# fgnt/pb_bss

Measured on NVIDIA H100. Metric: EM iterations/s, cACGMM F=513 T=500 D=8 K=3 (100-iteration fit), higher is better.
Workload: dtype f64

## Files before the change

### pb_bss_b200/csrc/em_persistent.cuh

```cuda
#pragma once
#include "common.cuh"
#include "em_kernels.cuh"
#include "heig.cuh"

namespace pbb {

#ifdef PBB_PHASE_TIMING
#define PBB_PH(i) do { if (tid == 0) { long long _t = clock64(); atomicAdd(&a.phase[i], (unsigned long long)(_t - _tp)); _tp = _t; } } while (0)
#else
#define PBB_PH(i) do { } while (0)
#endif

struct PersistArgs {
  const void* z;
  int zs;
  int F, T;
  int iterations;
  int first_is_m;
  int user_model;
  int softmax_fast;
  const double* aff_in;
  const double* saliency;
  const uint8_t* activity;
  double aff_eps;
  double eigenvalue_floor;
  int covariance_norm;
  int weight_mode;
  double* coef;
  double* ld;
  double* w;
  double* ew;
  double* part;
  int* flags;
  int* ticket;
  const int* dead;
  int* status;
  CwSpline spline;
  int wave_c;
  int wait_load;
  const int* order;
  unsigned long long* phase;
  int tsplit;
  double* tpart;
  int* tcount;
};

__device__ __forceinline__ uint32_t smem_u32(const void* p) {
  return static_cast<uint32_t>(__cvta_generic_to_shared(p));
}
__device__ __forceinline__ void mbar_init(uint64_t* bar, int count) {
  asm volatile("mbarrier.init.shared::cta.b64 [%0], %1;" ::"r"(smem_u32(bar)), "r"(count) : "memory");
}
__device__ __forceinline__ void mbar_expect_tx(uint64_t* bar, uint32_t bytes) {
  asm volatile("mbarrier.arrive.expect_tx.shared::cta.b64 _, [%0], %1;" ::"r"(smem_u32(bar)), "r"(bytes)
               : "memory");
}
__device__ __forceinline__ void mbar_wait(uint64_t* bar, uint32_t parity) {
  asm volatile(
      "{\n"
      ".reg .pred p;\n"
      "WAIT_%=:\n"
      "mbarrier.try_wait.parity.shared::cta.b64 p, [%0], %1;\n"
      "@p bra DONE_%=;\n"
      "bra WAIT_%=;\n"
      "DONE_%=:\n"
      "}\n" ::"r"(smem_u32(bar)),
      "r"(parity)
      : "memory");
}
__device__ __forceinline__ void bulk_g2s(void* dst, const void* src, uint32_t bytes, uint64_t* bar) {
  asm volatile("cp.async.bulk.shared::cluster.global.mbarrier::complete_tx::bytes [%0], [%1], %2, [%3];" ::"r"(
                   smem_u32(dst)),
               "l"(src), "r"(bytes), "r"(smem_u32(bar))
               : "memory");
}

constexpr int kStageFrames = 128;

template <int D, typename CT>
__device__ __forceinline__ void stage_g2s(CT (*dst)[kStageFrames], const CT* z, int bin, int nchunks, int chunk,
                                          uint64_t* bar) {
  constexpr int ROWS = stage_rows(D);
  constexpr uint32_t kRowBytes = kStageFrames * sizeof(CT);
  const CT* src = z + ((size_t)bin * nchunks + chunk) * (D * kStageFrames);
  mbar_expect_tx(bar, ROWS * kRowBytes);
  bulk_g2s(dst[0], src, D * kRowBytes, bar);
#pragma unroll
  for (int r = D; r < ROWS; ++r) bulk_g2s(dst[r], src + row_channel(D, r) * kStageFrames, kRowBytes, bar);
}

__device__ __forceinline__ int ld_acquire_gpu(const int* p) {
  int v;
  asm volatile("ld.acquire.gpu.global.s32 %0, [%1];" : "=r"(v) : "l"(p) : "memory");
  return v;
}
__device__ __forceinline__ void st_release_gpu(int* p, int v) {
  asm volatile("st.release.gpu.global.s32 [%0], %1;" ::"l"(p), "r"(v) : "memory");
}
__device__ __forceinline__ double fast_rcp(double x) {
  double r;
  asm("rcp.approx.ftz.f64 %0, %1;" : "=d"(r) : "d"(x));
  double e = fma(-x, r, 1.0);
  r = fma(r, e, r);
  e = fma(-x, r, 1.0);
  r = fma(r, e, r);
  return r;
}

__device__ __forceinline__ long long wave_h(long long r, int F, int c) {
  const long long m = F / c;
  const long long n = r < m ? r : m;
  return (long long)c * n * (n + 1) / 2 + (r - n) * (long long)F;
}
__device__ __forceinline__ long long wave_prefix(int r, int F, int I, int c) {
  return wave_h(r, F, c) - wave_h(r > I ? r - I : 0, F, c);
}
__device__ __forceinline__ void decode_ticket(int t, int F, int I, int c, int& bin, int& it) {
  if (c == 0) {
    it = t / F;
    bin = t - it * F;
    return;
  }
  int lo = 0, hi = I + (F + c - 1) / c - 1;
  while (hi - lo > 1) {
    const int mid = (lo + hi) >> 1;
    if (wave_prefix(mid, F, I, c) <= (long long)t) lo = mid; else hi = mid;
  }
  const long long first = (long long)c * (lo - I + 1 > 0 ? lo - I + 1 : 0);
  bin = (int)(first < F ? first : F) + (int)(t - wave_prefix(lo, F, I, c));
  it = lo - bin / c;
}
__device__ __forceinline__ int order_entry(const PersistArgs& a, int t, int S) {
  return a.order != nullptr ? __ldcg(a.order + t / S) : 0;
}
__device__ __forceinline__ void decode_task(const PersistArgs& a, int t, int S, int ord, int& bin, int& it, int& part) {
  const int tt = t / S;
  part = t - tt * S;
  if (a.order != nullptr) {
    bin = ord & 0xffff;
    it = ord >> 16;
  } else {
    decode_ticket(tt, a.F, a.iterations, a.wave_c, bin, it);
  }
}

__device__ __forceinline__ double2 lds_cplx(const double2* p) { return *p; }
__device__ __forceinline__ double2 lds_cplx(const float2* p) {
  const float2 v = *p;
  return make_double2((double)v.x, (double)v.y);
}

constexpr int kStages = 2;

template <int D, int K, typename CT>
struct PersistSmem {
  static constexpr int NS = D * D;
  static constexpr int M = D / 2;
  static constexpr int ROWS = stage_rows(D);
  CT zbuf[kStages][ROWS][kStageFrames];
  double2 A[K][NS];
  double2 V[K][NS];
  double2 W[K][NS];
  double coef[2][K][NS];
  double xq[2][M][2 * K][32];
  double S[K][NS + 1];
  alignas(16) double rot[K][((D + 1) / 2) * 6];
  double lam[K][D];
  double ld[K], w[K];
  alignas(16) double ew[2][4];
  alignas(16) double raw[2][8];
  uint64_t full[kStages];
  int tab[NS];
  int tick[8];
  int ready;
};

template <int D>
struct GroupDims {
  static constexpr int NSG = group_shape(D).nsg, NLOC = group_shape(D).nloc, NS = D * D;
  static constexpr int NFULL = group_shape(D).nfull, HALF = group_shape(D).half, M = D / 2;
};

template <int D>
__device__ __forceinline__ void group_psi(const double2 (&x)[GroupDims<D>::NLOC], double (&psi)[GroupDims<D>::NSG]) {
  using G = GroupDims<D>;
  psi[0] = x[0].x * x[0].x + x[0].y * x[0].y;
  psi[1] = x[1].x * x[1].x + x[1].y * x[1].y;
  psi[2] = x[0].x * x[1].x + x[0].y * x[1].y;
  psi[3] = x[0].x * x[1].y - x[0].y * x[1].x;
#pragma unroll
  for (int j = 0; j < G::NFULL; ++j) {
#pragma unroll
    for (int q = 0; q < 4; ++q) {
      const double2 u = x[q / 2], v = x[2 + 2 * j + (q % 2)];
      psi[4 + 8 * j + 2 * q] = u.x * v.x + u.y * v.y;
      psi[4 + 8 * j + 2 * q + 1] = u.x * v.y - u.y * v.x;
    }
  }
  if (G::HALF) {
#pragma unroll
    for (int h = 0; h < 2; ++h) {
      const double2 u = x[h], v = x[2 + 2 * G::NFULL + h];
      psi[4 + 8 * G::NFULL + 2 * h] = u.x * v.x + u.y * v.y;
      psi[4 + 8 * G::NFULL + 2 * h + 1] = u.x * v.y - u.y * v.x;
    }
  }
}

template <int D, int K>
__device__ __forceinline__ void softmax_product(double (&q)[K], const double* __restrict__ ew, double eps,
                                                double (&gam)[K], double (&cw)[K]) {
  const bool dead = q[0] < 1e-200;
#pragma unroll
  for (int k = 0; k < K; ++k) q[k] = dead ? 1.0 : q[k];
  double P[K];
  if constexpr (K == 2) {
    P[0] = q[1]; P[1] = q[0];
  } else if constexpr (K == 3) {
    P[0] = q[1] * q[2]; P[1] = q[0] * q[2]; P[2] = q[0] * q[1];
  } else {
    const double q01 = q[0] * q[1], q23 = q[2] * q[3];
    P[0] = q[1] * q23; P[1] = q[0] * q23; P[2] = q01 * q[3]; P[3] = q01 * q[2];
  }
  double b[K];
  double S = 1e-300;
#pragma unroll
  for (int k = 0; k < K; ++k) {
    b[k] = ew[k] * ipow<D>(P[k]);
    S += b[k];
  }
  const double rS = fast_rcp(S);
  const double rQ = fast_rcp(q[0] * P[0]);
  const double hi = 1.0 - eps;
#pragma unroll
  for (int k = 0; k < K; ++k) {
    double g = b[k] * rS;
    if (eps != 0.0) {
      g = g < eps ? eps : g;
      g = g > hi ? hi : g;
    }
    gam[k] = g;
    cw[k] = g * (P[k] * rQ);
  }
}

template <int K>
__device__ __forceinline__ void softmax_watson(const double (&q)[K], const double* __restrict__ kappa,
                                               const double* __restrict__ lognorm, const double* __restrict__ w,
                                               double (&gam)[K], double (&cw)[K]) {
  double lp[K];
  double m = -INFINITY;
#pragma unroll
  for (int k = 0; k < K; ++k) {
    lp[k] = fma(kappa[k], q[k], -lognorm[k]);
    m = lp[k] > m ? lp[k] : m;
  }
  double den = 0.0;
#pragma unroll
  for (int k = 0; k < K; ++k) {
    gam[k] = exp(lp[k] - m) * w[k];
    den += gam[k];
  }
  const double inv = 1.0 / fmax(den, kTiny);
#pragma unroll
  for (int k = 0; k < K; ++k) {
    gam[k] *= inv;
    cw[k] = gam[k];
  }
}

template <int D, bool NAMED>
__device__ __forceinline__ void em_exchange_barrier() {
  if constexpr (NAMED) asm volatile("bar.sync 1, %0;" ::"n"(32 * (D / 2)) : "memory");
  else __syncthreads();
}

template <int D, int K, int FR, typename CT>
__device__ __forceinline__ void lean_partial_forms(const CT* __restrict__ zrow, const double* __restrict__ cg,
                                                   double* __restrict__ xw, double (&psi)[FR][GroupDims<D>::NSG]) {
  using G = GroupDims<D>;
  constexpr int NSG = G::NSG, NLOC = G::NLOC, NS = G::NS;
  {
    double2 x[NLOC];
#pragma unroll
    for (int f = 0; f < FR; ++f) {
#pragma unroll
      for (int l = 0; l < NLOC; ++l) x[l] = lds_cplx(zrow + l * kStageFrames + 32 * f);
      group_psi<D>(x, psi[f]);
    }
  }
  double p0[FR][K], p1[FR][K];
#pragma unroll
  for (int k = 0; k < K; ++k)
#pragma unroll
    for (int f = 0; f < FR; ++f) { p0[f][k] = 0.0; p1[f][k] = 0.0; }
#pragma unroll
  for (int i = 0; i < NSG; i += 2) {
#pragma unroll
    for (int k = 0; k < K; ++k) {
      const double2 cc = *reinterpret_cast<const double2*>(cg + k * NS + i);
#pragma unroll
      for (int f = 0; f < FR; ++f) p0[f][k] = fma(cc.x, psi[f][i], p0[f][k]);
#pragma unroll
      for (int f = 0; f < FR; ++f) p1[f][k] = fma(cc.y, psi[f][i + 1], p1[f][k]);
    }
  }
#pragma unroll
  for (int k = 0; k < K; ++k)
#pragma unroll
    for (int f = 0; f < FR; ++f) xw[(f * K + k) * 32] = p0[f][k] + p1[f][k];
}

template <int D, int K, typename CT, int MODEL, bool NAMED = false, typename SMT>
__device__ __forceinline__ void lean_step(SMT& sm, int cb, int g, int st, int j, int lane, int& buf, double eps,
                                          double (&acc)[K * GroupDims<D>::NSG], double (&sg)[K]) {
  using G = GroupDims<D>;
  constexpr int NSG = G::NSG, M = G::M;
  double psi[1][NSG];
  lean_partial_forms<D, K, 1, CT>(&sm.zbuf[st][2 * g][0] + lane + 32 * j, &sm.coef[cb][0][g * NSG],
                                  &sm.xq[buf][g][0][lane], psi);
  em_exchange_barrier<D, NAMED>();
  const double* __restrict__ xr = &sm.xq[buf][0][0][lane];
  double q[K];
#pragma unroll
  for (int k = 0; k < K; ++k) {
    double v = xr[k * 32];
#pragma unroll
    for (int gg = 1; gg < M; ++gg) v += xr[(gg * 2 * K + k) * 32];
    q[k] = fabs(v);
  }
  buf ^= 1;
  double gam[K], cw[K];
  if constexpr (MODEL == 1) softmax_watson<K>(q, sm.ew[cb], sm.ld, sm.w, gam, cw);
  else softmax_product<D, K>(q, sm.ew[cb], eps, gam, cw);
#pragma unroll
  for (int k = 0; k < K; ++k) {
    sg[k] += gam[k];
#pragma unroll
    for (int i = 0; i < NSG; ++i) acc[k * NSG + i] = fma(cw[k], psi[0][i], acc[k * NSG + i]);
  }
}

template <int D, int K, typename CT, int MODEL, bool NAMED = false, typename SMT>
__device__ __forceinline__ void lean_chunk2(SMT& sm, int cb, int g, int st, int nsteps2, int lane,
                                            int& buf, double eps, double (&acc)[K * GroupDims<D>::NSG],
                                            double (&sg)[K]) {
  using G = GroupDims<D>;
  constexpr int NSG = G::NSG, M = G::M;
  const CT* __restrict__ zrow = &sm.zbuf[st][2 * g][0] + lane;
  const double* __restrict__ cg = &sm.coef[cb][0][g * NSG];
#pragma unroll 1
  for (int j = 0; j < nsteps2; ++j, zrow += 64) {
    double psi[2][NSG];
    lean_partial_forms<D, K, 2, CT>(zrow, cg, &sm.xq[buf][g][0][lane], psi);
    em_exchange_barrier<D, NAMED>();
    const double* __restrict__ xr = &sm.xq[buf][0][0][lane];
    double qA[K], qB[K];
#pragma unroll
    for (int k = 0; k < K; ++k) {
      double va = xr[k * 32], vb = xr[(K + k) * 32];
#pragma unroll
      for (int gg = 1; gg < M; ++gg) {
        va += xr[(gg * 2 * K + k) * 32];
        vb += xr[(gg * 2 * K + K + k) * 32];
      }
      qA[k] = fabs(va);
      qB[k] = fabs(vb);
    }
    buf ^= 1;
    double gA[K], cA[K], gB[K], cB[K];
    if constexpr (MODEL == 1) {
      softmax_watson<K>(qA, sm.ew[cb], sm.ld, sm.w, gA, cA);
      softmax_watson<K>(qB, sm.ew[cb], sm.ld, sm.w, gB, cB);
    } else {
      softmax_product<D, K>(qA, sm.ew[cb], eps, gA, cA);
      softmax_product<D, K>(qB, sm.ew[cb], eps, gB, cB);
    }
#pragma unroll
    for (int k = 0; k < K; ++k) {
      sg[k] += gA[k] + gB[k];
#pragma unroll
      for (int i = 0; i < NSG; ++i) {
        acc[k * NSG + i] = fma(cA[k], psi[0][i], acc[k * NSG + i]);
        acc[k * NSG + i] = fma(cB[k], psi[1][i], acc[k * NSG + i]);
      }
    }
  }
}

template <int D, int K, typename CT, typename SMT>
__device__ __forceinline__ void lean_chunk2_split(SMT& sm, int cb, int g, int st, int nsteps2, int lane, double eps,
                                                  double (&acc)[K * GroupDims<D>::NSG], double (&sg)[K]) {
  using G = GroupDims<D>;
  constexpr int NSG = G::NSG, M = G::M;
  static_assert(M == 4, "frame split assumes four slot-group warps");
  const CT* __restrict__ zrow = &sm.zbuf[st][2 * g][0] + lane;
  const double* __restrict__ cg = &sm.coef[cb][0][g * NSG];
  const int fsel = 16 * g + (lane & 15);
  const int fhalf = fsel >> 5, fl = fsel & 31;
#pragma unroll 1
  for (int j = 0; j < nsteps2; ++j, zrow += 64) {
    double psi[2][NSG];
    lean_partial_forms<D, K, 2, CT>(zrow, cg, &sm.xq[0][g][0][lane], psi);
    em_exchange_barrier<D, true>();
    {
      const double* __restrict__ xr = &sm.xq[0][0][fhalf * K][fl];
      double q[K];
#pragma unroll
      for (int k = 0; k < K; ++k) {
        double v = xr[k * 32];
#pragma unroll
        for (int gg = 1; gg < M; ++gg) v += xr[(gg * 2 * K + k) * 32];
        q[k] = fabs(v);
      }
      double gm[K], cw[K];
      softmax_product<D, K>(q, sm.ew[cb], eps, gm, cw);
#pragma unroll
      for (int k = 0; k < K; ++k) {
        sg[k] += lane < 16 ? gm[k] : 0.0;
        sm.cwx[k][fsel] = cw[k];
      }
    }
    em_exchange_barrier<D, true>();
    double cA[K], cB[K];
#pragma unroll
    for (int k = 0; k < K; ++k) {
      cA[k] = sm.cwx[k][lane];
      cB[k] = sm.cwx[k][32 + lane];
    }
#pragma unroll
    for (int k = 0; k < K; ++k) {
#pragma unroll
      for (int i = 0; i < NSG; ++i) acc[k * NSG + i] = fma(cA[k], psi[0][i], acc[k * NSG + i]);
#pragma unroll
      for (int i = 0; i < NSG; ++i) acc[k * NSG + i] = fma(cB[k], psi[1][i], acc[k * NSG + i]);
    }
  }
}

template <int D, int K>
__device__ __forceinline__ void softmax_general(const double (&q)[K], const double* __restrict__ ld,
                                                const double* __restrict__ w, const double* __restrict__ ew,
                                                bool fast, double eps, double (&gam)[K], double (&invq)[K]) {
  double a[K];
  if (fast) {
    double qmin = q[0];
#pragma unroll
    for (int k = 1; k < K; ++k) qmin = fmin(qmin, q[k]);
#pragma unroll
    for (int k = 0; k < K; ++k) {
      invq[k] = fast_rcp(q[k]);
      a[k] = ew[k] * ipow<D>(qmin * invq[k]);
    }
  } else {
    double lp[K];
    double m = -INFINITY;
#pragma unroll
    for (int k = 0; k < K; ++k) {
      lp[k] = -(double)D * log(q[k]) - ld[k];
      m = fmax(m, lp[k]);
      invq[k] = 1.0 / q[k];
    }
#pragma unroll
    for (int k = 0; k < K; ++k) a[k] = exp(lp[k] - m) * w[k];
  }
  double den = a[0];
#pragma unroll
  for (int k = 1; k < K; ++k) den += a[k];
  const double inv = 1.0 / fmax(den, kTiny);
#pragma unroll
  for (int k = 0; k < K; ++k) {
    double g = a[k] * inv;
    if (eps != 0.0) g = fmin(fmax(g, eps), 1.0 - eps);
    gam[k] = g;
  }
}

template <int D, int K, typename CT, bool FULL, bool NAMED = false, typename SMT>
__device__ __forceinline__ void general_chunk(const PersistArgs& a, SMT& sm, int g, int bin,
                                              int st, int t_chunk, int nsteps, int lane, int& buf, bool mstep_only,
                                              bool fast, double (&acc)[K * GroupDims<D>::NSG], double (&sg)[K]) {
  using G = GroupDims<D>;
  constexpr int NSG = G::NSG, NLOC = G::NLOC, M = G::M, NS = G::NS;
  const int T = a.T;
  const CT* __restrict__ zb = &sm.zbuf[st][0][0];
  const CT* __restrict__ zg = zb + 2 * g * kStageFrames + lane;
#pragma unroll 1
  for (int j = 0; j < nsteps; ++j) {
    const int t = t_chunk + j * 32 + lane;
    const bool valid = t < T;
    const int tc = valid ? t : 0;
    double2 x[NLOC];
#pragma unroll
    for (int l = 0; l < NLOC; ++l) x[l] = lds_cplx(zg + l * kStageFrames + j * 32);
    double psi[NSG];
    group_psi<D>(x, psi);
    double gam[K], invq[K];
    bool done = false;
    if constexpr (FULL) {
      if (!mstep_only) {
        const double* __restrict__ cg = &sm.coef[0][0][g * NSG];
#pragma unroll
        for (int k = 0; k < K; ++k) {
          double pq = 0.0;
#pragma unroll
          for (int i = 0; i < NSG; ++i) pq = fma(cg[k * NS + i], psi[i], pq);
          sm.xq[buf][g][k][lane] = pq;
        }
        em_exchange_barrier<D, NAMED>();
        double q[K];
#pragma unroll
        for (int k = 0; k < K; ++k) {
          double v = sm.xq[buf][0][k][lane];
#pragma unroll
          for (int gg = 1; gg < M; ++gg) v += sm.xq[buf][gg][k][lane];
          q[k] = fmax(fabs(v), 10.0 * kTiny);
        }
        buf ^= 1;
        if (a.activity != nullptr) {
          double ewm[K], wm[K];
#pragma unroll
          for (int k = 0; k < K; ++k) {
            const bool on = a.activity[((size_t)bin * K + k) * T + tc] != 0;
            ewm[k] = on ? sm.ew[0][k] : 0.0;
            wm[k] = on ? sm.w[k] : 0.0;
          }
          softmax_general<D, K>(q, sm.ld, wm, ewm, fast, a.aff_eps, gam, invq);
        } else {
          softmax_general<D, K>(q, sm.ld, sm.w, sm.ew[0], fast, a.aff_eps, gam, invq);
        }
        done = true;
      }
    }
    if (!done) {
#pragma unroll
      for (int k = 0; k < K; ++k) {
        gam[k] = __ldcg(a.aff_in + ((size_t)bin * K + k) * T + tc);
        invq[k] = 1.0;
      }
    }
    double sal = 1.0;
    if (FULL && a.saliency != nullptr) sal = a.saliency[(size_t)bin * T + tc];
#pragma unroll
    for (int k = 0; k < K; ++k) {
      const double gs = valid ? gam[k] * sal : 0.0;
      const double cw = gs * invq[k];
      sg[k] += gs;
#pragma unroll
      for (int i = 0; i < NSG; ++i) acc[k * NSG + i] = fma(cw, psi[i], acc[k * NSG + i]);
    }
  }
}

template <int D>
__device__ __forceinline__ double warp_hpd_inverse(double2* __restrict__ A, int lane, bool* ok) {
  constexpr int NS = D * D;
  constexpr int PER = (NS + 31) / 32;
  int ri[PER], ci[PER];
  double2 mine[PER];
#pragma unroll
  for (int r = 0; r < PER; ++r) {
    const int idx = lane + 32 * r;
    ri[r] = idx / D;
    ci[r] = idx - ri[r] * D;
    mine[r] = idx < NS ? A[idx] : make_double2(0.0, 0.0);
  }
  double det = 1.0;
  bool good = true;
#pragma unroll 1
  for (int j = 0; j < D; ++j) {
    const double p = A[j * D + j].x;
    good = good && (p > 0.0) && (p < 1e300);
    const double ip = fast_rcp(p);
    det *= p;
#pragma unroll
    for (int r = 0; r < PER; ++r) {
      if (lane + 32 * r < NS) {
        const int i = ri[r], k = ci[r];
        const double2 aij = A[i * D + j], ajk = A[j * D + k];
        const double sx = aij.x * ip, sy = aij.y * ip;
        double2 v = make_double2(mine[r].x - (sx * ajk.x - sy * ajk.y), mine[r].y - (sx * ajk.y + sy * ajk.x));
        if (k == j) v = make_double2(-sx, -sy);
        if (i == j) v = make_double2(ajk.x * ip, ajk.y * ip);
        if (i == j && k == j) v = make_double2(ip, 0.0);
        mine[r] = v;
      }
    }
    __syncwarp();
#pragma unroll
    for (int r = 0; r < PER; ++r)
      if (lane + 32 * r < NS) A[lane + 32 * r] = mine[r];
    __syncwarp();
  }
  *ok = good;
  return det;
}

template <int D, bool FULL>
__device__ __forceinline__ void cacg_update_class(const PersistArgs& a, int bin, int k, int K, int lane,
                                                  double2* __restrict__ A, double2* __restrict__ V,
                                                  double* __restrict__ lamk, const double* __restrict__ Sk,
                                                  const int* __restrict__ tab, double* __restrict__ ld_out,
                                                  double* __restrict__ coef_out = nullptr) {
  constexpr int NS = D * D;
  double* Ad = reinterpret_cast<double*>(A);
    const int dead_bin = a.dead == nullptr ? 0 : __ldcg(a.dead + bin);
#ifdef PBB_PHASE_TIMING
    long long _tu = clock64();
#define PBB_PHU(i) do { if (k == 0 && lane == 0) { long long _t = clock64(); atomicAdd(&a.phase[i], (unsigned long long)(_t - _tu)); _tu = _t; } } while (0)
#else
#define PBB_PHU(i) do { } while (0)
#endif
    const double scale = (double)D / fmax(Sk[NS], kTiny);
    bool bad = false;
    auto build_scaled = [&](double f) {
      for (int s = lane; s < NS; s += 32) {
        const int pk = tab[s];
        const int d = pk & 255, e = (pk >> 8) & 255, kind = pk >> 16;
        const double v = Sk[s] * f;
        bad |= !isfinite(v);
        if (kind == 0) { Ad[2 * (d * D + d)] = v; Ad[2 * (d * D + d) + 1] = 0.0; }
        else if (kind == 1) { Ad[2 * (d * D + e)] = v; Ad[2 * (e * D + d)] = v; }
        else { Ad[2 * (d * D + e) + 1] = -v; Ad[2 * (e * D + d) + 1] = v; }
      }
      __syncwarp();
    };
    auto build = [&]() { build_scaled(scale); };
    double tr, tn;
    if (a.covariance_norm == PBB_NORM_NONE) {
      build();
      tr = 0.0;
      for (int d = lane; d < D; d += 32) tr += A[d * D + d].x;
      tr = warp_sum(tr);
      tn = 1.0;
    } else {
      double trs = 0.0;
#pragma unroll
      for (int d = 0; d < D; ++d) trs += Sk[(d >> 1) * (NS / (D / 2)) + (d & 1)];
      tr = trs * scale;
      tn = (double)D / fmax(tr, kTiny);
      build_scaled(scale * tn);
    }
    PBB_PHU(8);
    bool ok;
    const double det = warp_hpd_inverse<D>(A, lane, &ok);
    PBB_PHU(9);
    double ldk = log(det);
    double tinv = 0.0;
    bool diag_pos = true;
#pragma unroll
    for (int d = 0; d < D; ++d) {
      tinv += A[d * D + d].x;
      diag_pos = diag_pos && A[d * D + d].x > 0.0;
    }
    const bool no_floor = ok && diag_pos && isfinite(tinv) && (tr * tn * tinv * a.eigenvalue_floor < 0.5) &&
                          dead_bin == 0;
    double* __restrict__ co = coef_out != nullptr ? coef_out : a.coef + ((size_t)bin * K + k) * NS;
    PBB_PHU(10);
    if (__any_sync(0xffffffffu, bad)) {
      if (lane == 0) atomicMax(a.status, bin + 1);
    }
    if (no_floor) {
      for (int s = lane; s < NS; s += 32) {
        const int pk = tab[s];
        const int d = pk & 255, e = (pk >> 8) & 255, kind = pk >> 16;
        const double2 u = A[d * D + e], v = A[e * D + d];
        co[s] = kind == 0 ? u.x : (kind == 1 ? (u.x + v.x) : -(u.y - v.y));
      }
    } else {
      build();
      if (a.covariance_norm == PBB_NORM_TRACE) {
        for (int i = lane; i < NS; i += 32) { A[i].x *= tn / D; A[i].y *= tn / D; }
        __syncwarp();
      }
      warp_jacobi_small<D>(A, V, lane);
      double lmax = -INFINITY;
      for (int d = lane; d < D; d += 32) lmax = fmax(lmax, A[d * D + d].x);
#pragma unroll
      for (int o = 16; o > 0; o >>= 1) lmax = fmax(lmax, __shfl_xor_sync(0xffffffffu, lmax, o));
      for (int d = lane; d < D; d += 32) {
        double l = A[d * D + d].x;
        if (a.covariance_norm == PBB_NORM_EIGENVALUE) l = fmax(l / fmax(lmax, kTiny), a.eigenvalue_floor);
        else l = fmax(l, lmax * a.eigenvalue_floor);
        if (!isfinite(l)) atomicMax(a.status, bin + 1);
        lamk[d] = l;
      }
      __syncwarp();
      ldk = model_from_eig_warp(V, lamk, tab, D, lane, co);
    }
    if (lane == 0) {
      *ld_out = ldk;
      if (!FULL) {
        a.ld[(size_t)bin * 4 + k] = ldk;
        a.ew[(size_t)bin * 4 + k] = Sk[NS];
      }
    }
    PBB_PHU(11);
}

template <int K>
__device__ __forceinline__ double lean_ew(double sgam, double ldk, const double* ld, int weight_mode, int T) {
  double ldmin = ld[0];
#pragma unroll
  for (int j = 1; j < K; ++j) ldmin = fmin(ldmin, ld[j]);
  const double wk = weight_mode == PBB_WEIGHT_CONST ? 1.0 / K : sgam / (double)T;
  return wk * exp(ldmin - ldk);
}

template <int D, int K, int MODEL, typename SMT>
__device__ __forceinline__ void padded_gamma(const SMT& sm, int cb, double eps, double (&gp)[K]) {
  double q[K], cw[K];
#pragma unroll
  for (int k = 0; k < K; ++k) q[k] = 0.0;
  if constexpr (MODEL == 1) softmax_watson<K>(q, sm.ew[cb], sm.ld, sm.w, gp, cw);
  else softmax_product<D, K>(q, sm.ew[cb], eps, gp, cw);
}

template <int D, int K>
__device__ __forceinline__ void store_group_sums(const double (&acc)[K * GroupDims<D>::NSG], int g, int lane,
                                                 double (*S)[D * D + 1]) {
  constexpr int NSG = GroupDims<D>::NSG;
  int lo, hi;
  reduce_range<K * NSG>(lane, lo, hi);
#pragma unroll
  for (int j = 0; j < HalvingSizes<K * NSG>::n5; ++j) {
    const int idx = lo + j;
    if (idx < hi) {
      const int k = idx / NSG, i = idx - k * NSG;
      S[k][g * NSG + i] = acc[j];
    }
  }
}

__device__ __forceinline__ bool split_last_part(const PersistArgs& a, int bin, int it, int S) {
  const int old = atomicAdd(a.tcount + bin, 1);
  __threadfence();
  return old + 1 == (it + 1) * S;
}
// ... 312 lines not shown
```

### pb_bss_b200/csrc/em_sticky.cuh

```cuda
#pragma once
#include <cooperative_groups.h>

#include "em_ws.cuh"

namespace pbb {

constexpr int kStickyEmRegs = 200;

__device__ __forceinline__ void sticky_cluster_sync() {
  asm volatile("barrier.cluster.arrive.release.aligned;\n\tbarrier.cluster.wait.acquire.aligned;" ::: "memory");
}

template <int K, typename CT>
__global__ void __launch_bounds__(256, 2) em_sticky_kernel(const PersistArgs a) {
  constexpr int D = 8;
  using SM = WsSmem<D, K, CT>;
  using G = GroupDims<D>;
  constexpr int NS = D * D, M = D / 2, NSG = G::NSG;
  constexpr int NU = K < 3 ? K : 3;
  extern __shared__ __align__(128) unsigned char smem_raw[];
  SM& sm = *reinterpret_cast<SM*>(smem_raw);
  namespace cg = cooperative_groups;
  cg::cluster_group cluster = cg::this_cluster();
  const int S = (int)cluster.num_blocks(), part = (int)cluster.block_rank();
  const int bin = blockIdx.x / S;
  const int tid = threadIdx.x, warp = tid >> 5, lane = tid & 31;
  const int zs = a.zs;
  const int nchunks = (zs + kStageFrames - 1) / kStageFrames;
  const int c0 = part * nchunks / S, c1 = (part + 1) * nchunks / S;

  for (int s = tid; s < NS; s += blockDim.x) sm.tab[s] = slot_pack(D, s);
  if (tid == 0) {
    for (int s = 0; s < kWsStages; ++s) mbar_init(&sm.full[s], 1);
    asm volatile("fence.mbarrier_init.release.cluster;" ::: "memory");
  }
  __syncthreads();
  if (tid == 0) {
    const CT* __restrict__ zbase = reinterpret_cast<const CT*>(a.z);
    for (int c = c0; c < c1; ++c) stage_g2s<D>(sm.zbuf[c - c0], zbase, bin, nchunks, c, &sm.full[c - c0]);
  }

  if (warp < M) {
    asm volatile("setmaxnreg.inc.sync.aligned.u32 %0;" ::"n"(kStickyEmRegs));
    const int g = warp;
#pragma unroll 1
    for (int it = 0; it < a.iterations; ++it) {
      const bool mstep_only = a.first_is_m && it == 0;
      double acc[K * NSG];
#pragma unroll
      for (int i = 0; i < K * NSG; ++i) acc[i] = 0.0;
      double sg[K];
#pragma unroll
      for (int k = 0; k < K; ++k) sg[k] = 0.0;
#pragma unroll 1
      for (int c = c0; c < c1; ++c) {
        const int st = c - c0;
        mbar_wait(&sm.full[st], 0u);
        ws_stage<K, CT>(a, sm, 0, g, bin, st, c, lane, mstep_only, acc, sg);
      }
      ws_task_end<K, CT>(a, sm, 0, g, c1, nchunks, lane, mstep_only, sg);
      warp_reduce_halving<K * NSG>(acc, lane);
      store_group_sums<D, K>(acc, g, lane, sm.S[0]);
#pragma unroll
      for (int k = 0; k < K; ++k) {
        const double v = warp_sum(sg[k]);
        if (lane == 0) sm.sgp[0][g][k] = v;
      }
      sticky_cluster_sync();
      sticky_cluster_sync();
      if (it + 1 < a.iterations) {
        if (tid < K) sm.ew[0][tid] = lean_ew<K>(sm.S[1][tid][NS], sm.ld[tid], sm.ld, a.weight_mode, a.T);
        asm volatile("bar.sync 1, %0;" ::"n"(32 * M) : "memory");
      }
    }
  } else {
    asm volatile("setmaxnreg.dec.sync.aligned.u32 %0;" ::"n"(256 - kStickyEmRegs));
    const int u = warp - M - 1;
#pragma unroll 1
    for (int it = 0; it < a.iterations; ++it) {
      sticky_cluster_sync();
      if (part == 0 && u >= 0 && u < NU) {
        const bool last_it = it == a.iterations - 1;
        for (int k = u; k < K; k += NU) {
          for (int i = lane; i < NS + 1; i += 32) {
            double v = 0.0;
            for (int p = 0; p < S; ++p) {
              if (i < NS) {
                v += *cluster.map_shared_rank(&sm.S[0][k][i], p);
              } else {
                const double* sp = cluster.map_shared_rank(&sm.sgp[0][0][k], p);
                v += (sp[0] + sp[K]) + (sp[2 * K] + sp[3 * K]);
              }
            }
            sm.S[1][k][i] = v;
          }
        }
        __syncwarp();
        if (last_it) {
          double* __restrict__ po = a.part + (size_t)bin * K * (NS + 1);
          for (int k = u; k < K; k += NU)
            for (int i = lane; i < NS + 1; i += 32) po[k * (NS + 1) + i] = sm.S[1][k][i];
        } else {
          for (int k = u; k < K; k += NU) {
            cacg_update_class<D, false>(a, bin, k, K, lane, sm.A[k], sm.V[k], sm.lam[k], sm.S[1][k], sm.tab, &sm.ld[k],
                                        &sm.coef[1][k][0]);
            __syncwarp();
            const double c0v = sm.coef[1][k][lane], c1v = sm.coef[1][k][lane + 32];
            const double ldk = sm.ld[k], sgam = sm.S[1][k][NS];
            for (int p = 0; p < S; ++p) {
              double* rc = cluster.map_shared_rank(&sm.coef[0][k][0], p);
              rc[lane] = c0v;
              rc[lane + 32] = c1v;
              if (lane == 0 && p != 0) {
                *cluster.map_shared_rank(&sm.ld[k], p) = ldk;
                *cluster.map_shared_rank(&sm.S[1][k][NS], p) = sgam;
              }
            }
          }
        }
      }
      sticky_cluster_sync();
    }
  }
}

}
```

### pb_bss_b200/csrc/em_ws.cuh

```cuda
#pragma once
#include "em_persistent.cuh"

namespace pbb {

constexpr int kWsLead = 2;
constexpr int kWsStages = 3;
constexpr int kWsEmRegs = 208;
constexpr int kWsHelperRegs = 256 - kWsEmRegs;

__device__ __forceinline__ void mbar_arrive(uint64_t* bar) {
  asm volatile("mbarrier.arrive.shared::cta.b64 _, [%0];" ::"r"(smem_u32(bar)) : "memory");
}

__device__ __forceinline__ void mbar_wait_relaxed(uint64_t* bar, uint32_t parity, unsigned ns) {
  while (true) {
    uint32_t done;
    asm volatile(
        "{\n"
        ".reg .pred p;\n"
        "mbarrier.try_wait.parity.shared::cta.b64 p, [%1], %2;\n"
        "selp.u32 %0, 1, 0, p;\n"
        "}\n"
        : "=r"(done)
        : "r"(smem_u32(bar)), "r"(parity)
        : "memory");
    if (done) break;
    __nanosleep(ns);
  }
}

template <int D, int K, typename CT>
struct WsSmem {
  static constexpr int NS = D * D;
  static constexpr int M = D / 2;
  static constexpr int ROWS = stage_rows(D);
  CT zbuf[kWsStages][ROWS][kStageFrames];
  double2 A[K][NS];
  double2 V[K][NS];
  double coef[2][K][NS];
  double xq[2][M][2 * K][32];
  double cwx[K][64];
  double sgp[2][M][K];
  double S[2][K][NS + 1];
  double lam[K][D];
  double ld[K];
  alignas(16) double ew[2][4];
  int tab[NS];
  int desc[2][4];
  int sdesc[2][4];
  int tlast;
  uint64_t full[kWsStages], empty[kWsStages];
  uint64_t model_full[2], model_empty[2];
  uint64_t s_full[2], s_empty[2];
};

template <int K, typename CT>
__device__ __forceinline__ void ws_stage(const PersistArgs& a, WsSmem<8, K, CT>& sm, int mb, int g, int bin, int st,
                                         int c, int lane, bool mstep_only,
                                         double (&acc)[K * GroupDims<8>::NSG], double (&sg)[K]) {
  constexpr int D = 8;
  const int t_chunk = c * kStageFrames;
  const int nsteps = (min(kStageFrames, a.zs - t_chunk)) >> 5;
  int buf = 0;
  if (!mstep_only) {
    lean_chunk2_split<D, K, CT>(sm, mb, g, st, nsteps >> 1, lane, a.aff_eps, acc, sg);
    if (nsteps & 1) {
      double sgt[K];
#pragma unroll
      for (int k = 0; k < K; ++k) sgt[k] = 0.0;
      lean_step<D, K, CT, 0, true>(sm, mb, g, st, nsteps - 1, lane, buf, a.aff_eps, acc, sgt);
#pragma unroll
      for (int k = 0; k < K; ++k) sg[k] += g == 0 ? sgt[k] : 0.0;
    }
  } else {
    general_chunk<D, K, CT, false>(a, sm, g, bin, st, t_chunk, nsteps, lane, buf, true, true, acc, sg);
  }
}

template <int K, typename CT>
__device__ __forceinline__ void ws_task_end(const PersistArgs& a, const WsSmem<8, K, CT>& sm, int mb, int g, int c1,
                                            int nchunks, int lane, bool mstep_only, double (&sg)[K]) {
  if (!mstep_only && a.zs > a.T && c1 == nchunks) {
    double gp[K];
    padded_gamma<8, K, 0>(sm, mb, a.aff_eps, gp);
    const int npad_lane = (g == 0 && lane >= 32 - (a.zs - a.T)) ? 1 : 0;
#pragma unroll
    for (int k = 0; k < K; ++k) sg[k] -= npad_lane ? gp[k] : 0.0;
  }
  if (mstep_only && g != 0) {
#pragma unroll
    for (int k = 0; k < K; ++k) sg[k] = 0.0;
  }
}

template <int K, typename CT>
__global__ void __launch_bounds__(256, 2) em_ws_kernel(const PersistArgs a) {
  constexpr int D = 8;
  using SM = WsSmem<D, K, CT>;
  using G = GroupDims<D>;
  constexpr int NS = D * D, M = D / 2, NSG = G::NSG;
  constexpr int NU = K < 3 ? K : 3;
  extern __shared__ __align__(128) unsigned char smem_raw[];
  SM& sm = *reinterpret_cast<SM*>(smem_raw);
  const int tid = threadIdx.x, warp = tid >> 5, lane = tid & 31;
  const int F = a.F, T = a.T, zs = a.zs;
  const int nchunks = (zs + kStageFrames - 1) / kStageFrames;
  const int S = a.tsplit > 1 ? a.tsplit : 1;
  const int total = a.iterations * F * S;

  for (int s = tid; s < NS; s += blockDim.x) sm.tab[s] = slot_pack(D, s);
  if (tid == 0) {
    for (int s = 0; s < kWsStages; ++s) { mbar_init(&sm.full[s], 1); mbar_init(&sm.empty[s], M); }
    for (int s = 0; s < 2; ++s) {
      mbar_init(&sm.model_full[s], 1);
      mbar_init(&sm.model_empty[s], M);
      mbar_init(&sm.s_full[s], M);
      mbar_init(&sm.s_empty[s], NU);
    }
    asm volatile("fence.mbarrier_init.release.cluster;" ::: "memory");
  }
  __syncthreads();

  if (warp < M) {
    asm volatile("setmaxnreg.inc.sync.aligned.u32 %0;" ::"n"(kWsEmRegs));
    const int g = warp;
    unsigned chunk_cnt = 0;
#ifdef PBB_PHASE_TIMING
    long long _tp = clock64();
#endif
#pragma unroll 1
    for (unsigned n = 0;; ++n) {
      const int mb = n & 1;
      mbar_wait(&sm.model_full[mb], (n >> 1) & 1u);
      PBB_PH(0);
      const int bin = sm.desc[mb][0], it = sm.desc[mb][1], part = sm.desc[mb][2];
      const int c0 = part * nchunks / S, c1 = (part + 1) * nchunks / S;
      if (bin < 0) {
        const int sb = n & 1;
        mbar_wait(&sm.s_empty[sb], ((n >> 1) & 1u) ^ 1u);
        if (lane == 0) {
          if (g == 0) sm.sdesc[sb][0] = -1;
          mbar_arrive(&sm.s_full[sb]);
        }
        break;
      }
      const bool mstep_only = a.first_is_m && it == 0;
      double acc[K * NSG];
#pragma unroll
      for (int i = 0; i < K * NSG; ++i) acc[i] = 0.0;
      double sg[K];
#pragma unroll
      for (int k = 0; k < K; ++k) sg[k] = 0.0;
#pragma unroll 1
      for (int c = c0; c < c1; ++c) {
        const int st = chunk_cnt % kWsStages;
        mbar_wait(&sm.full[st], (chunk_cnt / kWsStages) & 1u);
        PBB_PH(2);
        ws_stage<K, CT>(a, sm, mb, g, bin, st, c, lane, mstep_only, acc, sg);
        __syncwarp();
        if (lane == 0) mbar_arrive(&sm.empty[st]);
        ++chunk_cnt;
        PBB_PH(3);
      }
      ws_task_end<K, CT>(a, sm, mb, g, c1, nchunks, lane, mstep_only, sg);
      __syncwarp();
      if (lane == 0) mbar_arrive(&sm.model_empty[mb]);

      warp_reduce_halving<K * NSG>(acc, lane);
      const int sb = n & 1;
      PBB_PH(4);
      mbar_wait(&sm.s_empty[sb], ((n >> 1) & 1u) ^ 1u);
      PBB_PH(5);
      store_group_sums<D, K>(acc, g, lane, sm.S[sb]);
#pragma unroll
      for (int k = 0; k < K; ++k) {
        const double v = warp_sum(sg[k]);
        if (lane == 0) sm.sgp[sb][g][k] = v;
      }
      if (g == 0 && lane == 0) { sm.sdesc[sb][0] = bin; sm.sdesc[sb][1] = it; sm.sdesc[sb][2] = part; }
      __syncwarp();
      if (lane == 0) mbar_arrive(&sm.s_full[sb]);
      PBB_PH(6);
    }
  } else {
    asm volatile("setmaxnreg.dec.sync.aligned.u32 %0;" ::"n"(kWsHelperRegs));
    if (warp == M) {
      const CT* __restrict__ zbase = reinterpret_cast<const CT*>(a.z);
      unsigned chunk_cnt = 0;
#pragma unroll 1
      for (unsigned n = 0;; ++n) {
        const int mb = n & 1;
        int t = 0;
        if (lane == 0) t = atomicAdd(a.ticket, 1);
        t = __shfl_sync(0xffffffffu, t, 0);
        int bin = -1, it = 0, part = 0;
        if (t < total) decode_task(a, t, S, order_entry(a, t, S), bin, it, part);
        const int c0 = part * nchunks / S, ncp = (part + 1) * nchunks / S - c0;
        const bool mstep_only = a.first_is_m && it == 0;
        int issued = 0;
        auto issue_chunks = [&](int upto, bool blocking) {
          while (issued < upto) {
            const int st = chunk_cnt % kWsStages;
            const uint32_t par = ((chunk_cnt / kWsStages) & 1u) ^ 1u;
            if (blocking) {
              mbar_wait_relaxed(&sm.empty[st], par, 100);
            } else {
              uint32_t done;
              asm volatile(
                  "{\n"
                  ".reg .pred p;\n"
                  "mbarrier.test_wait.parity.shared::cta.b64 p, [%1], %2;\n"
                  "selp.u32 %0, 1, 0, p;\n"
                  "}\n"
                  : "=r"(done)
                  : "r"(smem_u32(&sm.empty[st])), "r"(par)
                  : "memory");
              if (!done) break;
            }
            stage_g2s<D>(sm.zbuf[st], zbase, bin, nchunks, c0 + issued, &sm.full[st]);
            ++chunk_cnt;
            ++issued;
          }
        };
        if (bin >= 0 && lane == 0) {
          bool z_ready = !a.wait_load;
          if (!z_ready && ld_acquire_gpu(a.flags + bin) >= 0) {
            asm volatile("fence.proxy.async;" ::: "memory");
            z_ready = true;
          }
          if (z_ready) issue_chunks(ncp, false);
          if (mstep_only) {
            if (a.wait_load) while (ld_acquire_gpu(a.flags + bin) < 0) __nanosleep(200);
          } else {
            while (ld_acquire_gpu(a.flags + bin) < it) {
              if (z_ready) issue_chunks(ncp, false);
              __nanosleep(40);
            }
          }
          if (!z_ready) asm volatile("fence.proxy.async;" ::: "memory");
        }
        __syncwarp();
        mbar_wait_relaxed(&sm.model_empty[mb], ((n >> 1) & 1u) ^ 1u, 100);
        if (bin >= 0 && !mstep_only) {
          const double* __restrict__ cf = a.coef + (size_t)bin * K * NS;
          for (int i = lane; i < K * NS; i += 32) (&sm.coef[mb][0][0])[i] = __ldcg(cf + i);
          if (lane < K) {
            double ld[K];
#pragma unroll
            for (int j = 0; j < K; ++j) ld[j] = __ldcg(a.ld + (size_t)bin * 4 + j);
            sm.ew[mb][lane] = lean_ew<K>(__ldcg(a.ew + (size_t)bin * 4 + lane), __ldcg(a.ld + (size_t)bin * 4 + lane),
                                         ld, a.weight_mode, T);
          }
        }
        if (lane == 0) { sm.desc[mb][0] = bin; sm.desc[mb][1] = it; sm.desc[mb][2] = part; }
        __syncwarp();
        if (lane == 0) mbar_arrive(&sm.model_full[mb]);
        if (bin < 0) break;
        if (lane == 0) {
          issue_chunks(ncp, true);
          const unsigned x = chunk_cnt - (unsigned)(ncp >= kWsLead + 1 ? kWsLead + 1 : ncp);
          mbar_wait_relaxed(&sm.empty[x % kWsStages], (x / kWsStages) & 1u, 100);
        }
        __syncwarp();
      }
    } else if (warp - M - 1 < NU) {
      const int u = warp - M - 1;
#ifdef PBB_PHASE_TIMING
      long long _tp = clock64();
#undef PBB_PH
#define PBB_PH(i) do { if (u == 0 && lane == 0) { long long _t = clock64(); atomicAdd(&a.phase[i], (unsigned long long)(_t - _tp)); _tp = _t; } } while (0)
#endif
#pragma unroll 1
      for (unsigned n = 0;; ++n) {
        const int sb = n & 1;
        mbar_wait_relaxed(&sm.s_full[sb], (n >> 1) & 1u, 100);
        PBB_PH(7);
        const int bin = sm.sdesc[sb][0], it = sm.sdesc[sb][1];
        if (bin < 0) break;
        const bool last_it = it == a.iterations - 1;
        for (int k = u; k < K; k += NU)
          if (lane == 0)
            sm.S[sb][k][NS] = (sm.sgp[sb][0][k] + sm.sgp[sb][1][k]) + (sm.sgp[sb][2][k] + sm.sgp[sb][3][k]);
        __syncwarp();
        if (last_it && S == 1) asm volatile("bar.sync 2, %0;" ::"n"(NU * 32) : "memory");
        if (S > 1) {
          const int part = sm.sdesc[sb][2];
          constexpr int kRow = K * (NS + 1);
          double* __restrict__ tp = a.tpart + ((size_t)bin * S + part) * kRow;
          for (int k = u; k < K; k += NU)
            for (int i = lane; i < NS + 1; i += 32) __stcg(tp + k * (NS + 1) + i, sm.S[sb][k][i]);
          __threadfence();
          asm volatile("bar.sync 2, %0;" ::"n"(NU * 32) : "memory");
          if (u == 0 && lane == 0) sm.tlast = split_last_part(a, bin, it, S);
          asm volatile("bar.sync 2, %0;" ::"n"(NU * 32) : "memory");
          if (!sm.tlast) {
            __syncwarp();
            if (lane == 0) mbar_arrive(&sm.s_empty[sb]);
            continue;
          }
          for (int k = u; k < K; k += NU)
            for (int i = lane; i < NS + 1; i += 32) sm.S[sb][k][i] = split_sum<D, K>(a, bin, S, k * (NS + 1) + i);
          __syncwarp();
          if (last_it) asm volatile("bar.sync 2, %0;" ::"n"(NU * 32) : "memory");
        }
        if (last_it) {
          double* __restrict__ po = a.part + (size_t)bin * K * (NS + 1);
          for (int i = u * 32 + lane; i < K * (NS + 1); i += NU * 32) po[i] = (&sm.S[sb][0][0])[i];
        } else {
          for (int k = u; k < K; k += NU)
            cacg_update_class<D, false>(a, bin, k, K, lane, sm.A[k], sm.V[k], sm.lam[k], sm.S[sb][k], sm.tab, &sm.ld[k]);
        }
        __syncwarp();
        if (lane == 0) mbar_arrive(&sm.s_empty[sb]);
        if (!last_it) {
          asm volatile("bar.sync 2, %0;" ::"n"(NU * 32) : "memory");
          if (u == 0 && lane == 0) st_release_gpu(a.flags + bin, it + 1);
        }
        PBB_PH(1);
      }
    }
  }
}

}
```

Baseline: 41530.

## Skew E/M steps across double-buffered exchange slots in sticky kernel

In the sticky cluster kernel, the two 64-frame steps of a ring stage are now software-pipelined. Both partial-form passes write to separate xq buffers, and the cwx exchange buffer is doubled, so fewer named barriers are needed per stage. The M-step reloads the frames from shared memory and recomputes psi instead of holding it in registers across the barriers, trading extra shared loads and FMAs for lower register pressure. The warp-specialized path keeps the old schedule, and the odd-tail step now uses buffer 1 to avoid clobbering buffer 0.

```diff
diff --git a/pb_bss_b200/csrc/em_persistent.cuh b/pb_bss_b200/csrc/em_persistent.cuh
--- a/pb_bss_b200/csrc/em_persistent.cuh
+++ b/pb_bss_b200/csrc/em_persistent.cuh
@@ -275,20 +275,23 @@
   else __syncthreads();
 }
 
+template <int D, int FR, typename CT>
+__device__ __forceinline__ void load_group_psi(const CT* __restrict__ zrow, double (&psi)[FR][GroupDims<D>::NSG]) {
+  double2 x[GroupDims<D>::NLOC];
+#pragma unroll
+  for (int f = 0; f < FR; ++f) {
+#pragma unroll
+    for (int l = 0; l < GroupDims<D>::NLOC; ++l) x[l] = lds_cplx(zrow + l * kStageFrames + 32 * f);
+    group_psi<D>(x, psi[f]);
+  }
+}
+
 template <int D, int K, int FR, typename CT>
 __device__ __forceinline__ void lean_partial_forms(const CT* __restrict__ zrow, const double* __restrict__ cg,
                                                    double* __restrict__ xw, double (&psi)[FR][GroupDims<D>::NSG]) {
   using G = GroupDims<D>;
-  constexpr int NSG = G::NSG, NLOC = G::NLOC, NS = G::NS;
-  {
-    double2 x[NLOC];
-#pragma unroll
-    for (int f = 0; f < FR; ++f) {
-#pragma unroll
-      for (int l = 0; l < NLOC; ++l) x[l] = lds_cplx(zrow + l * kStageFrames + 32 * f);
-      group_psi<D>(x, psi[f]);
-    }
-  }
+  constexpr int NSG = G::NSG, NS = G::NS;
+  load_group_psi<D, FR, CT>(zrow, psi);
   double p0[FR][K], p1[FR][K];
 #pragma unroll
   for (int k = 0; k < K; ++k)
@@ -388,52 +391,85 @@
   }
 }
 
-template <int D, int K, typename CT, typename SMT>
+template <int D, int K, bool SKEW, typename CT, typename SMT>
 __device__ __forceinline__ void lean_chunk2_split(SMT& sm, int cb, int g, int st, int nsteps2, int lane, double eps,
                                                   double (&acc)[K * GroupDims<D>::NSG], double (&sg)[K]) {
   using G = GroupDims<D>;
   constexpr int NSG = G::NSG, M = G::M;
   static_assert(M == 4, "frame split assumes four slot-group warps");
+  static_assert(kStageFrames == 128, "a ring stage is at most two steps of 64 frames (xq / cwx hold two)");
   const CT* __restrict__ zrow = &sm.zbuf[st][2 * g][0] + lane;
   const double* __restrict__ cg = &sm.coef[cb][0][g * NSG];
   const int fsel = 16 * g + (lane & 15);
   const int fhalf = fsel >> 5, fl = fsel & 31;
+  auto posterior = [&](int b) {
+    const double* __restrict__ xr = &sm.xq[b][0][fhalf * K][fl];
+    double q[K];
+#pragma unroll
+    for (int k = 0; k < K; ++k) {
+      double v = xr[k * 32];
+#pragma unroll
+      for (int gg = 1; gg < M; ++gg) v += xr[(gg * 2 * K + k) * 32];
+      q[k] = fabs(v);
+    }
+    double gm[K], cw[K];
+    softmax_product<D, K>(q, sm.ew[cb], eps, gm, cw);
+#pragma unroll
+    for (int k = 0; k < K; ++k) {
+      sg[k] += lane < 16 ? gm[k] : 0.0;
+      sm.cwx[b][k][fsel] = cw[k];
+    }
+  };
+  auto mstep = [&](const double (&psi)[2][NSG], int b) {
+    double cA[K], cB[K];
+#pragma unroll
+    for (int k = 0; k < K; ++k) {
+      cA[k] = sm.cwx[b][k][lane];
+      cB[k] = sm.cwx[b][k][32 + lane];
+    }
+#pragma unroll
+    for (int k = 0; k < K; ++k) {
+#pragma unroll
+      for (int i = 0; i < NSG; ++i) acc[k * NSG + i] = fma(cA[k], psi[0][i], acc[k * NSG + i]);
+#pragma unroll
+      for (int i = 0; i < NSG; ++i) acc[k * NSG + i] = fma(cB[k], psi[1][i], acc[k * NSG + i]);
+    }
+  };
+  if constexpr (!SKEW) {
 #pragma unroll 1
-  for (int j = 0; j < nsteps2; ++j, zrow += 64) {
-    double psi[2][NSG];
-    lean_partial_forms<D, K, 2, CT>(zrow, cg, &sm.xq[0][g][0][lane], psi);
+    for (int j = 0; j < nsteps2; ++j, zrow += 64) {
+      double psi[2][NSG];
+      lean_partial_forms<D, K, 2, CT>(zrow, cg, &sm.xq[0][g][0][lane], psi);
+      em_exchange_barrier<D, true>();
+      posterior(0);
+      em_exchange_barrier<D, true>();
+      mstep(psi, 0);
+    }
+  } else {
+    auto estep = [&](int j) {
+      double psi[2][NSG];
+      lean_partial_forms<D, K, 2, CT>(zrow + 64 * j, cg, &sm.xq[j][g][0][lane], psi);
+    };
+    auto mstep_recomputed = [&](int j) {
+      double psi[2][NSG];
+      load_group_psi<D, 2, CT>(zrow + 64 * j, psi);
+      mstep(psi, j);
+    };
+    if (nsteps2 == 0) return;
+    estep(0);
     em_exchange_barrier<D, true>();
-    {
-      const double* __restrict__ xr = &sm.xq[0][0][fhalf * K][fl];
-      double q[K];
-#pragma unroll
-      for (int k = 0; k < K; ++k) {
-        double v = xr[k * 32];
-#pragma unroll
-        for (int gg = 1; gg < M; ++gg) v += xr[(gg * 2 * K + k) * 32];
-        q[k] = fabs(v);
-      }
-      double gm[K], cw[K];
-      softmax_product<D, K>(q, sm.ew[cb], eps, gm, cw);
-#pragma unroll
-      for (int k = 0; k < K; ++k) {
-        sg[k] += lane < 16 ? gm[k] : 0.0;
-        sm.cwx[k][fsel] = cw[k];
-      }
-    }
-    em_exchange_barrier<D, true>();
-    double cA[K], cB[K];
-#pragma unroll
-    for (int k = 0; k < K; ++k) {
-      cA[k] = sm.cwx[k][lane];
-      cB[k] = sm.cwx[k][32 + lane];
-    }
-#pragma unroll
-    for (int k = 0; k < K; ++k) {
-#pragma unroll
-      for (int i = 0; i < NSG; ++i) acc[k * NSG + i] = fma(cA[k], psi[0][i], acc[k * NSG + i]);
-#pragma unroll
-      for (int i = 0; i < NSG; ++i) acc[k * NSG + i] = fma(cB[k], psi[1][i], acc[k * NSG + i]);
+    if (nsteps2 == 2) {
+      estep(1);
+      posterior(0);
+      em_exchange_barrier<D, true>();
+      mstep_recomputed(0);
+      posterior(1);
+      em_exchange_barrier<D, true>();
+      mstep_recomputed(1);
+    } else {
+      posterior(0);
+      em_exchange_barrier<D, true>();
+      mstep_recomputed(0);
     }
   }
 }
diff --git a/pb_bss_b200/csrc/em_sticky.cuh b/pb_bss_b200/csrc/em_sticky.cuh
--- a/pb_bss_b200/csrc/em_sticky.cuh
+++ b/pb_bss_b200/csrc/em_sticky.cuh
@@ -56,7 +56,7 @@
       for (int c = c0; c < c1; ++c) {
         const int st = c - c0;
         mbar_wait(&sm.full[st], 0u);
-        ws_stage<K, CT>(a, sm, 0, g, bin, st, c, lane, mstep_only, acc, sg);
+        ws_stage<K, CT, true>(a, sm, 0, g, bin, st, c, lane, mstep_only, acc, sg);
       }
       ws_task_end<K, CT>(a, sm, 0, g, c1, nchunks, lane, mstep_only, sg);
       warp_reduce_halving<K * NSG>(acc, lane);
diff --git a/pb_bss_b200/csrc/em_ws.cuh b/pb_bss_b200/csrc/em_ws.cuh
--- a/pb_bss_b200/csrc/em_ws.cuh
+++ b/pb_bss_b200/csrc/em_ws.cuh
@@ -39,7 +39,7 @@
   double2 V[K][NS];
   double coef[2][K][NS];
   double xq[2][M][2 * K][32];
-  double cwx[K][64];
+  double cwx[2][K][64];
   double sgp[2][M][K];
   double S[2][K][NS + 1];
   double lam[K][D];
@@ -54,16 +54,16 @@
   uint64_t s_full[2], s_empty[2];
 };
 
-template <int K, typename CT>
+template <int K, typename CT, bool SKEW>
 __device__ __forceinline__ void ws_stage(const PersistArgs& a, WsSmem<8, K, CT>& sm, int mb, int g, int bin, int st,
                                          int c, int lane, bool mstep_only,
                                          double (&acc)[K * GroupDims<8>::NSG], double (&sg)[K]) {
   constexpr int D = 8;
   const int t_chunk = c * kStageFrames;
   const int nsteps = (min(kStageFrames, a.zs - t_chunk)) >> 5;
-  int buf = 0;
+  int buf = 1;
   if (!mstep_only) {
-    lean_chunk2_split<D, K, CT>(sm, mb, g, st, nsteps >> 1, lane, a.aff_eps, acc, sg);
+    lean_chunk2_split<D, K, SKEW, CT>(sm, mb, g, st, nsteps >> 1, lane, a.aff_eps, acc, sg);
     if (nsteps & 1) {
       double sgt[K];
 #pragma unroll
@@ -156,7 +156,7 @@
         const int st = chunk_cnt % kWsStages;
         mbar_wait(&sm.full[st], (chunk_cnt / kWsStages) & 1u);
         PBB_PH(2);
-        ws_stage<K, CT>(a, sm, mb, g, bin, st, c, lane, mstep_only, acc, sg);
+        ws_stage<K, CT, false>(a, sm, mb, g, bin, st, c, lane, mstep_only, acc, sg);
         __syncwarp();
         if (lane == 0) mbar_arrive(&sm.empty[st]);
         ++chunk_cnt;
```

Result: no change. 41420, median of 6 (-0.3%).
